# allegro/allRank

Hardware: AMD Instinct MI355X
Metric: slate-items/sec training (WEB30K synth, slate 240) (higher is better)
Workload: dtype f32 (split-bf16x3 contractions: GEMMs and attention); 1 GPU; WEB30K-synth F=136 L=240, fc[512] + 2x self-attention(d512,h8,d_ff2048) + ApproxNDCG (BASELINE configs[2]); slates_per_gpu=256, slate_len=240, global_batch=256, optimizer=Adam lr=1e-3, slates=dense, engine=fused, gemm=split_bf16, parallelism=slate-sharded dp1

## Files before the change

### allrank_amd/csrc/ltrx_mha.hip

```cpp
#include "ltrx_mfma.h"

using namespace ltrx;

namespace {

template <int DKP>
struct Tile {
  static constexpr int LDT = DKP + 4;
  static constexpr int FLOATS = 32 * LDT;
};

template <int DKP>
__device__ __forceinline__ void stage_tile(float* tile, const float* __restrict__ base, int row0, int nrows, int dk,
                                           size_t rs) {
  constexpr int C4 = DKP / 4;
  for (int idx = threadIdx.x; idx < 32 * C4; idx += blockDim.x) {
    const int r = idx / C4, c = (idx % C4) * 4;
    float4 v = make_float4(0.f, 0.f, 0.f, 0.f);
    if (row0 + r < nrows && c < dk) v = *reinterpret_cast<const float4*>(base + (size_t)(row0 + r) * rs + c);
    *reinterpret_cast<float4*>(tile + r * Tile<DKP>::LDT + c) = v;
  }
}

template <int DKP>
// ... 334 lines not shown
      del_t[threadIdx.x] = (qrow < L) ? delta[statb + qrow] : 0.f;
      if (DROP) drow_t[threadIdx.x] = drop_row_seed(drop, bh, Lmax, qrow);
    }
    __syncthreads();
    if (qt + 1 < nqt) {
      tile_gload<DKP>(qr, qb, (qt + 1) * 32, L, dk, rs);
      tile_gload<DKP>(dor, dob, (qt + 1) * 32, L, dk, ors);
    }
    const f32x16 s = rows_x_fixed<DKP>(qtile, kfrag);
    f32x16 p;
#pragma unroll
    for (int r = 0; r < 16; ++r) p[r] = fast_exp2(s[r] * sl2 + kbias - lse_t[rowmap(r, half)]);
    f32x16 dm;
#pragma unroll
    for (int r = 0; r < 16; ++r)
      dm[r] = DROP ? drop_scale_rk(drop, drow_t[rowmap(r, half)], key) : 1.0f;
    {
      f32x16 pd;
#pragma unroll
      for (int r = 0; r < 16; ++r) pd[r] = p[r] * dm[r];
      cols_x_p<DKP>(dotile, pd, dvacc);
    }
    const f32x16 dp = rows_x_fixed<DKP>(dotile, vfrag);
    f32x16 ds;
#pragma unroll
    for (int r = 0; r < 16; ++r) ds[r] = p[r] * (dp[r] * dm[r] - del_t[rowmap(r, half)]) * scale;
    cols_x_p<DKP>(qtile, ds, dkacc);
  }
  store_rows<DKP>(dkout + slate * drs + (size_t)head * dk, k0, L, dk, drs, dkacc, 1.0f);
  store_rows<DKP>(dvout + slate * drs + (size_t)head * dk, k0, L, dk, drs, dvacc, 1.0f);
}

__global__ void ltrx_selftest_mfma_kernel(const float* __restrict__ A, const float* __restrict__ Bm, float* __restrict__ D) {
  const int lane = threadIdx.x & 63, half = lane >> 5;
  f32x16 acc = {0.f, 0.f, 0.f, 0.f, 0.f, 0.f, 0.f, 0.f, 0.f, 0.f, 0.f, 0.f, 0.f, 0.f, 0.f, 0.f};
  acc = __builtin_amdgcn_mfma_f32_32x32x2f32(A[(lane & 31) * 2 + half], Bm[half * 32 + (lane & 31)], acc, 0, 0, 0);
  for (int r = 0; r < 16; ++r) D[rowmap(r, half) * 32 + (lane & 31)] = acc[r];
}

extern "C" int ltrx_selftest_mfma32x32x2(const float* A, const float* Bm, float* D, ltrx_stream_t stream) {
  if (!A || !Bm || !D) return LTRX_EINVAL;
  hipLaunchKernelGGL(ltrx_selftest_mfma_kernel, dim3(1), dim3(64), 0, (hipStream_t)stream, A, Bm, D);
  LTRX_LAUNCH_CHECK();
  return LTRX_OK;
}

bool ltrx_mha_res_fits(int L, int dk);
int ltrx_mha_fwd_res_launch(const float* q, const float* k, const float* v, const uint8_t* kpm, int B, int L, int h, int dk, int rs,
                            float* o, int ors, float* lse, float p_drop, uint32_t seed, const uint32_t* seed_step, const int* cu,
                            const int* order, bool plain, hipStream_t s);
int ltrx_mha_bwd_res_launch(const float* q, const float* k, const float* v, const uint8_t* kpm, const float* o, const float* dout,
                            const float* lse, int B, int L, int h, int dk, int rs, int ors, float* dq, float* dkk, float* dv, int drs,
                            void* ws, float p_drop, uint32_t seed, const uint32_t* seed_step, const int* cu, const int* order,
                            bool plain, hipStream_t s);
bool ltrx_mha_res_bwd_fits(int L, int dk);
size_t ltrx_mha_res_bwd_ws_bytes(int B, int L, int h);

static int mha_check(int B, int L, int h, int dk, int rs, int ors) {
  if (B <= 0 || L <= 0 || h <= 0 || dk <= 0) return LTRX_EINVAL;
  if (dk % 4 != 0 || dk > 128 || rs % 4 != 0 || ors % 4 != 0 || rs < h * dk || ors < h * dk) return LTRX_EUNSUPPORTED;
  if ((long long)B * h > 0x7fffffffLL || (L + 127) / 128 > 65535) return LTRX_EUNSUPPORTED;
  return LTRX_OK;
}

extern "C" int ltrx_mha_head_width_supported(int d_k) { return mha_check(1, 1, 1, d_k, d_k, d_k) == LTRX_OK ? 1 : 0; }

#define LTRX_DKP_DISPATCH(dk, CALL) \
  do {                              \
    if ((dk) <= 32) { CALL(32); }   \
    else if ((dk) <= 64) { CALL(64); } \
    else if ((dk) <= 96) { CALL(96); } \
    else { CALL(128); }             \
  } while (0)

static DropCfg make_drop(float p_drop, uint32_t seed) { return ltrx_make_drop(p_drop, seed); }

extern "C" int ltrx_mha_fwd(const float* q, const float* k, const float* v, const uint8_t* key_pad_mask, int B, int L,
                            int h, int d_k, int row_stride, float* o, int o_row_stride, float* lse_out, float p_drop,
                            uint32_t seed, const uint32_t* seed_step, const int32_t* cu_seqlens, const int32_t* slate_order,
                            int mode, ltrx_stream_t stream) {
  if (!q || !k || !v || (!key_pad_mask && !cu_seqlens) || !o || !lse_out || !(p_drop >= 0.f) || p_drop >= 1.f) return LTRX_EINVAL;
  if (mode < 0 || mode > 2) return LTRX_EINVAL;
  int rc = mha_check(B, L, h, d_k, row_stride, o_row_stride);
  if (rc != LTRX_OK) return rc;
  hipStream_t s = (hipStream_t)stream;
  if (mode != 0 && ltrx_mha_res_fits(L, d_k))
    return ltrx_mha_fwd_res_launch(q, k, v, key_pad_mask, B, L, h, d_k, row_stride, o, o_row_stride, lse_out, p_drop, seed, seed_step,
                                   cu_seqlens, slate_order, mode == 2, s);
  const DropCfg drop = make_drop(p_drop, seed);
  const dim3 grid(B * h, (L + 127) / 128);
  const float scale = 1.0f / sqrtf((float)d_k);
#define CALL(DKP)                                                                                                 \
  if (drop.thresh != 0u)                                                                                          \
    hipLaunchKernelGGL((ltrx_mha_fwd_kernel<DKP, true>), grid, dim3(256), 0, s, q, k, v, key_pad_mask, L, h, d_k, row_stride, \
                       o, o_row_stride, lse_out, scale, drop, seed_step, cu_seqlens, slate_order);                              \
  else                                                                                                            \
    hipLaunchKernelGGL((ltrx_mha_fwd_kernel<DKP, false>), grid, dim3(256), 0, s, q, k, v, key_pad_mask, L, h, d_k, row_stride, \
                       o, o_row_stride, lse_out, scale, drop, seed_step, cu_seqlens, slate_order)
  LTRX_DKP_DISPATCH(d_k, CALL);
#undef CALL
  LTRX_LAUNCH_CHECK();
  return LTRX_OK;
}

static bool res_bwd_selected(int B, int L, int h, int d_k) {
  return ltrx_mha_res_bwd_fits(L, d_k) && ltrx_mha_res_bwd_ws_bytes(B, L, h) <= (size_t)LTRX_MHA_DS_BUDGET_BYTES;
}

extern "C" size_t ltrx_mha_bwd_workspace_bytes(int B, int L, int h, int d_k, int mode) {
  if (B <= 0 || L <= 0 || h <= 0 || d_k <= 0) return 0;
  if (mode != 0 && res_bwd_selected(B, L, h, d_k)) return ltrx_mha_res_bwd_ws_bytes(B, L, h);
  return (size_t)B * L * h * sizeof(float);
}

extern "C" int ltrx_mha_bwd(const float* q, const float* k, const float* v, const uint8_t* key_pad_mask, const float* o,
                            const float* dout, const float* lse, int B, int L, int h, int d_k, int row_stride,
                            int o_row_stride, float* dq, float* dk, float* dv, int d_row_stride, float p_drop,
                            uint32_t seed, const uint32_t* seed_step, const int32_t* cu_seqlens, const int32_t* slate_order,
                            int mode, void* ws, ltrx_stream_t stream) {
  if (!q || !k || !v || (!key_pad_mask && !cu_seqlens) || !o || !dout || !lse || !dq || !dk || !dv || !ws) return LTRX_EINVAL;
  if (mode < 0 || mode > 2) return LTRX_EINVAL;
  if (!(p_drop >= 0.f) || p_drop >= 1.f) return LTRX_EINVAL;
  int rc = mha_check(B, L, h, d_k, row_stride, o_row_stride);
  if (rc != LTRX_OK) return rc;
  if (d_row_stride % 4 != 0 || d_row_stride < h * d_k) return LTRX_EUNSUPPORTED;
  hipStream_t s = (hipStream_t)stream;
  float* delta = (float*)ws;
  if (mode != 0 && res_bwd_selected(B, L, h, d_k))
    return ltrx_mha_bwd_res_launch(q, k, v, key_pad_mask, o, dout, lse, B, L, h, d_k, row_stride, o_row_stride, dq, dk, dv, d_row_stride,
                                   ws, p_drop, seed, seed_step, cu_seqlens, slate_order, mode == 2, s);
  const DropCfg drop = make_drop(p_drop, seed);
  const dim3 grid(B * h, (L + 127) / 128);
  const float scale = 1.0f / sqrtf((float)d_k);
#define CALLQ(DKP)                                                                                                   \
  if (drop.thresh != 0u)                                                                                             \
    hipLaunchKernelGGL((ltrx_mha_bwd_dq_kernel<DKP, true>), grid, dim3(256), 0, s, q, k, v, key_pad_mask, o, dout, lse, delta, \
                       L, h, d_k, row_stride, o_row_stride, dq, d_row_stride, scale, drop, seed_step, cu_seqlens, slate_order);    \
  else                                                                                                               \
    hipLaunchKernelGGL((ltrx_mha_bwd_dq_kernel<DKP, false>), grid, dim3(256), 0, s, q, k, v, key_pad_mask, o, dout, lse, delta, \
                       L, h, d_k, row_stride, o_row_stride, dq, d_row_stride, scale, drop, seed_step, cu_seqlens, slate_order)
  LTRX_DKP_DISPATCH(d_k, CALLQ);
#undef CALLQ
  LTRX_LAUNCH_CHECK();
#define CALLK(DKP)                                                                                                     \
  if (drop.thresh != 0u)                                                                                               \
    hipLaunchKernelGGL((ltrx_mha_bwd_dkdv_kernel<DKP, true>), grid, dim3(256), 0, s, q, k, v, key_pad_mask, dout, lse, delta, L, \
                       h, d_k, row_stride, o_row_stride, dk, dv, d_row_stride, scale, drop, seed_step, cu_seqlens, slate_order);      \
  else                                                                                                                 \
    hipLaunchKernelGGL((ltrx_mha_bwd_dkdv_kernel<DKP, false>), grid, dim3(256), 0, s, q, k, v, key_pad_mask, dout, lse, delta, L, \
                       h, d_k, row_stride, o_row_stride, dk, dv, d_row_stride, scale, drop, seed_step, cu_seqlens, slate_order)
  LTRX_DKP_DISPATCH(d_k, CALLK);
#undef CALLK
  LTRX_LAUNCH_CHECK();
  return LTRX_OK;
}
```

### allrank_amd/csrc/ltrx_mha_res.hip

```cpp
#include "ltrx_mfma.h"

using namespace ltrx;

namespace {

constexpr int RMAX = 256;
constexpr int DK = 64;
constexpr int PLANE = RMAX * DK * 2;
constexpr size_t RES_STATS = 4 * (size_t)PLANE + 3 * RMAX * sizeof(float);
constexpr int XROW = 64;
constexpr size_t dq_smem(int nw) { return 2 * (size_t)PLANE + (size_t)nw * 32 * 32 * sizeof(float); }
constexpr float kLog2e = 1.4426950408889634f;
constexpr float kLn2 = 0.6931471805599453f;


__device__ __forceinline__ int img_off(int row, int chunk) {
  const int s = ((row >> 2) & 1) | (((row >> 3) & 1) << 1) | (((row >> 1) & 1) << 2);
  return row * (DK * 2) + ((chunk ^ s) << 4);
}

struct TileRegs {
  float4 a, b;
};
__device__ __forceinline__ void tile_gload(TileRegs& r, const float* __restrict__ base, int tile, int nrows, int dk, size_t rs) {
// ... 23 lines not shown
  f32x4 x[8];
};
__device__ __forceinline__ void fixed_gload(FixedRegs& f, const float* __restrict__ base, int row0, int nrows, int dk, size_t rs) {
  const int lane = threadIdx.x & 63, c16 = lane & 15;
#pragma unroll
  for (int j = 0; j < 8; ++j) {
    const int r = (lane >> 4) + 4 * j;
    const bool ok = (row0 + r < nrows) && (4 * c16 < dk);
    const f32x4 v = *reinterpret_cast<const f32x4*>(base + (size_t)(ok ? row0 + r : 0) * rs + (ok ? 4 * c16 : 0));
    f.x[j] = ok ? v : f32x4{0.f, 0.f, 0.f, 0.f};
  }
}
__device__ __forceinline__ void fixed_finish(bf16x8 (&fh)[4], bf16x8 (&fl)[4], const FixedRegs& f, f32x4* scratch, float pre = 1.0f) {
  const int lane = threadIdx.x & 63, l31 = lane & 31, half = lane >> 5, c16 = lane & 15;
#pragma unroll
  for (int j = 0; j < 8; ++j) {
    const int r = (lane >> 4) + 4 * j;
    scratch[r * 16 + (c16 ^ (r & 15))] = f.x[j];
  }
#pragma unroll
  for (int ks = 0; ks < 4; ++ks) {
    const f32x4 a = scratch[l31 * 16 + ((4 * ks + 2 * half) ^ (l31 & 15))];
    const f32x4 b = scratch[l31 * 16 + ((4 * ks + 2 * half + 1) ^ (l31 & 15))];
    const float v[8] = {a.x * pre, a.y * pre, a.z * pre, a.w * pre, b.x * pre, b.y * pre, b.z * pre, b.w * pre};
#pragma unroll
    for (int e = 0; e < 8; ++e) {
      LTRX_SPLIT_BF16(v[e], fh[ks][e], fl[ks][e]);
    }
  }
}

#define LTRX_MFMA(a, b, c) __builtin_amdgcn_mfma_f32_32x32x16_bf16(a, b, c, 0, 0, 0)
#ifdef LTRX_MHA_STAMP
__device__ unsigned long long g_mha_stamps[8][40][8];
#define STAMP_(kt, ph)                                                                 \
  do {                                                                                 \
    __builtin_amdgcn_sched_barrier(0);                                                 \
    if (blockIdx.x == LTRX_MHA_STAMP && (threadIdx.x & 63) == 0) g_mha_stamps[threadIdx.x >> 6][kt][ph] = __builtin_readcyclecounter(); \
    __builtin_amdgcn_sched_barrier(0);                                                 \
  } while (0)
#ifdef LTRX_MHA_STAMP_DKDV
#define STAMP(kt, ph)
#define DSTAMP(kt, ph) STAMP_(kt, ph)
#else
#define STAMP(kt, ph) STAMP_(kt, ph)
#define DSTAMP(kt, ph)
#endif
#else
#define STAMP(kt, ph)
#define DSTAMP(kt, ph)
#endif
#ifndef LTRX_MHA_TOUCH
#define LTRX_MHA_TOUCH 1
#endif
#ifndef LTRX_MHA_PRIO_HALF
#define LTRX_MHA_PRIO_HALF 0
#endif

struct ColFrags {
  bf16x8 h[2][2], l[2][2];
};
__device__ __forceinline__ void store_rows(float* __restrict__ base, int row0, int nrows, int dk, size_t rs, const f32x16 (&out)[2],
                                           float scale, f32x4* scratch) {
  const int lane = threadIdx.x & 63, l31 = lane & 31, half = lane >> 5;
#pragma unroll
  for (int ct = 0; ct < 2; ++ct) {
#pragma unroll
    for (int g = 0; g < 4; ++g)
      scratch[l31 * 8 + ((2 * g + half) ^ ((l31 >> 1) & 7))] =
          f32x4{out[ct][4 * g + 0] * scale, out[ct][4 * g + 1] * scale, out[ct][4 * g + 2] * scale, out[ct][4 * g + 3] * scale};
#pragma unroll
    for (int j = 0; j < 4; ++j) {
      const int r = (lane >> 3) + 8 * j, c = 32 * ct + 4 * (lane & 7);
      const f32x4 v = scratch[r * 8 + ((lane & 7) ^ ((r >> 1) & 7))];
      if (row0 + r < nrows && c < dk) *reinterpret_cast<f32x4*>(base + (size_t)(row0 + r) * rs + c) = v;
    }
  }
}
__device__ __forceinline__ f32x4* end_scratch(unsigned char* smem, int last_tile, int wave) {
  const size_t half_off = (((last_tile & 7) >= 4) ? 0 : PLANE / 2);
  return reinterpret_cast<f32x4*>(smem + (size_t)(wave >> 2) * PLANE + half_off + (size_t)(wave & 3) * 4096);
}

__device__ __forceinline__ void zero2(f32x16 (&o)[2]) {
#pragma unroll
  for (int ct = 0; ct < 2; ++ct)
#pragma unroll
    for (int r = 0; r < 16; ++r) o[ct][r] = 0.f;
}

struct Slate {
  int b, head, bh, Lmax, len;
  size_t row0;
};
__device__ __forceinline__ Slate which_slate(int L, int h, const int* __restrict__ cu, const int* __restrict__ order) {
  Slate s;
  s.head = blockIdx.x % h;
  s.b = order ? order[blockIdx.x / h] : (int)(blockIdx.x / h);
  s.bh = s.b * h + s.head;
  s.Lmax = L;
  s.row0 = cu ? (size_t)cu[s.b] : (size_t)s.b * L;
  s.len = cu ? cu[s.b + 1] - cu[s.b] : L;
  return s;
}

struct Touch {
// ... 225 lines not shown
    const float mref = (mn == -INFINITY) ? 0.f : mn;
    if (__builtin_amdgcn_ballot_w64(grow) != 0) {
      const float alpha = grow ? fast_exp2(m - mref) : 1.0f;
      l *= alpha;
#pragma unroll
      for (int ct = 0; ct < 2; ++ct)
#pragma unroll
        for (int r = 0; r < 16; ++r) oacc[ct][r] *= alpha;
    }
    m = mn;
    f32x16 p;
    f32x2 ps2 = {0.f, 0.f};
    const f32x2 mref2 = {mref, mref};
#pragma unroll
    for (int r = 0; r < 16; r += 2) {
      const f32x2 t = f32x2{s[r], s[r + 1]} - mref2;
      const f32x2 e2 = {fast_exp2(t[0]), fast_exp2(t[1])};
      ps2 += e2;
      p[r] = e2[0];
      p[r + 1] = e2[1];
    }
    l += ps2[0] + ps2[1];
    if (DROP) {
#pragma unroll
      for (int r = 0; r < 16; ++r) p[r] *= drop_scale_rk(drop, drow, kt * 32 + rowmap(r, half));
    }
    STAMP(kt, 4);
    cols_mma<PL>(vimg + slot * (DK * 2), fo, p, oacc);
    STAMP(kt, 5);
  }
  STAMP(33, 0);
  if (!active) {
    if (LTRX_MHA_TOUCH) touch_join(tch);
    return;
  }
  const float lt = sum_across_halves(l);
  const float inv = (lt > 0.f) ? 1.0f / lt : 0.f;
  store_rows(o + sl.row0 * ors + (size_t)sl.head * dk, q0, len, dk, ors, oacc, inv, end_scratch(smem, nkt - 1, wave));
  const int qrow = q0 + (lane & 31);
  if (half == 0 && qrow < len) lse[((size_t)sl.b * h + sl.head) * sl.Lmax + qrow] = (lt > 0.f) ? (m + log2f(lt)) * kLn2 : 0.f;
  STAMP(34, 0);
  if (LTRX_MHA_TOUCH) touch_join(tch);
}

struct DsRegs {
  f32x4 x[4];
};
__device__ __forceinline__ void ds_gload(DsRegs& d, const float* __restrict__ rows, int tile, int LK) {
  const int lane = threadIdx.x & 63;
  const float* p = rows + (size_t)(lane >> 3) * LK + tile * 32 + (lane & 7) * 4;
#pragma unroll
  for (int j = 0; j < 4; ++j) d.x[j] = __builtin_nontemporal_load(reinterpret_cast<const f32x4*>(p + (size_t)(8 * j) * LK));
}
template <bool PL, int NW, int D, bool KPF>
__global__ void __launch_bounds__(64 * NW) __attribute__((amdgpu_waves_per_eu(2, 2))) ltrx_mha_bwd_dq_res_kernel(const float* __restrict__ k, const float* __restrict__ dsw, int LK, int L,
                                                                  int h, int dk, int rs, float* __restrict__ dq, int drs,
                                                                  const int* __restrict__ cu, const int* __restrict__ order) {
  extern __shared__ __attribute__((aligned(16))) unsigned char smem[];
  unsigned char* kimg = smem;
  const Slate sl = which_slate(L, h, cu, order);
  const int lane = threadIdx.x & 63, half = lane >> 5, wave = __builtin_amdgcn_readfirstlane(threadIdx.x >> 6), l31 = lane & 31;
  f32x4* xs = reinterpret_cast<f32x4*>(smem + 2 * PLANE) + wave * (32 * 32 / 4);
  const int len = sl.len;
  constexpr int TPT = 32 / NW;
  if ((int)(blockIdx.y * (32 * NW)) >= len) return;
  const float* src = k + sl.row0 * rs + (size_t)sl.head * dk;
  const int q0 = blockIdx.y * (32 * NW) + wave * 32;
  const int sub = (NW == 8) ? (int)(threadIdx.x >> 8) : 0;
  const bool active = q0 < len;
  const float* rows = dsw + ((size_t)sl.b * h + sl.head) * LK * LK + (size_t)q0 * LK;
  const int nkt = (len + 31) / 32, nchunk = KPF ? (nkt + 7) / 8 : 1;
  static_assert(KPF ? (8 % D == 0) : true, "the register slot of tile 8 c + s must not depend on c");
  TileRegs tr[TPT];
#pragma unroll
  for (int j = 0; j < TPT; ++j) tile_gload(tr[j], src, (8 / TPT) * j + sub, len, dk, rs);
  DsRegs dr[D];
  if (active) {
#pragma unroll
    for (int s = 0; s < D; ++s)
      if (s < nkt) ds_gload(dr[s], rows, s, LK);
  }
  f32x16 dqacc[2];
  zero2(dqacc);
  const TileOffsets fo = tile_offsets();
  for (int c = 0; c < nchunk; ++c) {
    if (c > 0) lds_only_barrier();
#pragma unroll
    for (int j = 0; j < TPT; ++j) tile_sstore<PL>(kimg, (8 / TPT) * j + sub, tr[j]);
    if (KPF && c + 1 < nchunk) {
#pragma unroll
      for (int j = 0; j < TPT; ++j) tile_gload(tr[j], src, 8 * (c + 1) + (8 / TPT) * j + sub, len, dk, rs);
    }
    lds_only_barrier();
    if (!active) continue;
#pragma unroll
    for (int s = 0; s < 8; ++s) {
      const int i = 8 * c + s;
      if (i >= nkt) break;
      DsRegs& cur = dr[s % D];
#pragma unroll
      for (int j = 0; j < 4; ++j) {
        const int r = (lane >> 3) + 8 * j;
        xs[r * 8 + ((lane & 7) ^ ((r >> 1) & 7))] = cur.x[j];
      }
      if (i + D < nkt) ds_gload(cur, rows, i + D, LK);
      f32x16 ds;
#pragma unroll
      for (int g = 0; g < 4; ++g) {
        const f32x4 x = xs[l31 * 8 + ((2 * g + half) ^ ((l31 >> 1) & 7))];
        ds[4 * g + 0] = x.x;
        ds[4 * g + 1] = x.y;
        ds[4 * g + 2] = x.z;
        ds[4 * g + 3] = x.w;
      }
      cols_mma<PL>(kimg + s * 32 * (DK * 2), fo, ds, dqacc);
    }
  }
  if (!active) return;
  store_rows(dq + sl.row0 * drs + (size_t)sl.head * dk, q0, len, dk, drs, dqacc, 1.0f, xs);
}

__device__ __forceinline__ float tile_delta(const TileRegs& g, const TileRegs& a) {
  float d = g.a.x * a.a.x + g.a.y * a.a.y + g.a.z * a.a.z + g.a.w * a.a.w;
  d += g.b.x * a.b.x + g.b.y * a.b.y + g.b.z * a.b.z + g.b.w * a.b.w;
  d += __shfl_xor(d, 4, 64);
  d += __shfl_xor(d, 2, 64);
  d += __shfl_xor(d, 1, 64);
  return d;
}
template <bool DROP, bool PL>
__global__ void __launch_bounds__(512) ltrx_mha_bwd_dkdv_res_kernel(
    const float* __restrict__ q, const float* __restrict__ k, const float* __restrict__ v, const uint8_t* __restrict__ kpm,
    const float* __restrict__ o, const float* __restrict__ dout, const float* __restrict__ lse, int L, int h, int dk, int rs, int ors,
    float* __restrict__ dkout, float* __restrict__ dvout, int drs, float* __restrict__ dsw, int LK, float scale, DropCfg drop,
    const uint32_t* __restrict__ drop_step, const int* __restrict__ cu, const int* __restrict__ order) {
  extern __shared__ __attribute__((aligned(16))) unsigned char smem[];
  unsigned char* qimg = smem;
  unsigned char* doimg = smem + 2 * PLANE;
  float* lse_t = reinterpret_cast<float*>(smem + 4 * PLANE);
  float* del_t = lse_t + RMAX;
  uint32_t* drow_t = reinterpret_cast<uint32_t*>(del_t + RMAX);
  if (DROP && drop_step) drop.seed ^= drop_step[0] * 0x9E3779B9u;
  const Slate sl = which_slate(L, h, cu, order);
  const int lane = threadIdx.x & 63, half = lane >> 5, wave = __builtin_amdgcn_readfirstlane(threadIdx.x >> 6);
  const int len = sl.len;
  const bool first = wave < 4;
  const float* src = first ? q + sl.row0 * rs + (size_t)sl.head * dk : dout + sl.row0 * ors + (size_t)sl.head * dk;
  const float* osrc = o + sl.row0 * ors + (size_t)sl.head * dk;
  const size_t srs = first ? (size_t)rs : (size_t)ors;
  unsigned char* dst = first ? qimg : doimg;
  TileRegs tr, to;
  DSTAMP(32, 0);
  tile_gload(tr, src, 0, len, dk, srs);
  if (!first) tile_gload(to, osrc, 0, len, dk, ors);
  const size_t statb = ((size_t)sl.b * h + sl.head) * sl.Lmax;
  float lse_n = 0.f;
  if (threadIdx.x < 32 && (int)threadIdx.x < len) lse_n = lse[statb + threadIdx.x];
  if ((int)(blockIdx.y * RMAX) >= len) return;
  const int k0 = blockIdx.y * RMAX + wave * 32;
  bf16x8 kh[4], kl[4], vh[4], vl[4];
  const bool active = k0 < len;
  const int key = k0 + (lane & 31);
  bool key_masked;
  {
    FixedRegs fk, fv;
    fixed_gload(fk, k + sl.row0 * rs + (size_t)sl.head * dk, k0, len, dk, rs);
    fixed_gload(fv, v + sl.row0 * rs + (size_t)sl.head * dk, k0, len, dk, rs);
    const uint8_t km = kpm ? kpm[sl.row0 + (key < len ? key : 0)] : (uint8_t)0;
    f32x4* scratch = reinterpret_cast<f32x4*>(smem + (size_t)(wave >> 1) * PLANE + PLANE / 2 + (size_t)(wave & 1) * 8192);
    fixed_finish(kh, kl, fk, scratch, scale * kLog2e);
    fixed_finish(vh, vl, fv, scratch, scale);
    key_masked = (key >= len) || km != 0;
  }
  const float kbias = key_masked ? -INFINITY : 0.f;
  const f32x2 kb2 = {kbias, kbias};
  const TileOffsets fo = tile_offsets();
  f32x16 dkacc[2], dvacc[2];
  zero2(dkacc);
  zero2(dvacc);
  const int nqt = (len + 31) / 32;
  if (LTRX_MHA_PRIO_HALF && wave >= 4) __builtin_amdgcn_s_setprio(1);
  float* const dsp = dsw + ((size_t)sl.b * h + sl.head) * LK * LK + (blockIdx.y * RMAX + wave * 32);
  const int dso = (4 * half * LK + (lane & 31)) * 4;
  DSTAMP(32, 1);
  for (int qt = 0; qt < nqt; ++qt) {
    DSTAMP(qt, 0);
    if (!first) {
      const float d = tile_delta(tr, to);
// ... 4 lines not shown
      const int qr = qt * 32 + threadIdx.x, sl_ = (qt & 7) * 32 + threadIdx.x;
      lse_t[sl_] = (qr < len) ? lse_n * kLog2e : INFINITY;
      if (DROP) drow_t[sl_] = drop_row_seed(drop, sl.bh, sl.Lmax, qr);
    }
    DSTAMP(qt, 1);
    lds_only_barrier();
    DSTAMP(qt, 2);
    if (!active) {
      if (qt + 1 < nqt) {
        tile_gload(tr, src, qt + 1, len, dk, srs);
        if (!first) tile_gload(to, osrc, qt + 1, len, dk, ors);
      }
      continue;
    }
    const int slot = (qt & 7) * 32;
    const unsigned char* qtile = qimg + slot * (DK * 2);
    const unsigned char* dotile = doimg + slot * (DK * 2);
    f32x16 p = rows_mma<PL>(qtile, fo, kh, kl);
    f32x16 ds = rows_mma<PL>(dotile, fo, vh, vl);
    DSTAMP(qt, 3);
    {
      const float* lse_p = reinterpret_cast<const float*>(reinterpret_cast<const unsigned char*>(lse_t + slot) + fo.kb);
      const float* del_p = reinterpret_cast<const float*>(reinterpret_cast<const unsigned char*>(del_t + slot) + fo.kb);
#pragma unroll
      for (int g = 0; g < 4; ++g) {
        const f32x4 ls4 = *reinterpret_cast<const f32x4*>(lse_p + 8 * g);
        const f32x4 dl4 = *reinterpret_cast<const f32x4*>(del_p + 8 * g);
#pragma unroll
        for (int e = 0; e < 4; e += 2) {
          const int r = 4 * g + e;
          const f32x2 t = (f32x2{p[r], p[r + 1]} - f32x2{ls4[e], ls4[e + 1]}) + kb2;
          const f32x2 pr = {fast_exp2(t[0]), fast_exp2(t[1])};
          f32x2 dm = {1.0f, 1.0f};
          if (DROP) {
            const int qr = slot + rowmap(r, half);
            dm = f32x2{drop_scale_rk(drop, drow_t[qr], key), drop_scale_rk(drop, drow_t[qr + 1], key)};
          }
          const f32x2 dpv = {ds[r], ds[r + 1]};
          const f32x2 x = (DROP ? dpv * dm : dpv) - f32x2{dl4[e], dl4[e + 1]};
          const f32x2 dsv = pr * x;
          const f32x2 pm = DROP ? pr * dm : pr;
          ds[r] = dsv[0];
          ds[r + 1] = dsv[1];
          p[r] = pm[0];
          p[r + 1] = pm[1];
        }
      }
    }
    DSTAMP(qt, 4);
    {
      const float* const t = dsp + (size_t)(qt * 32) * LK;
#pragma unroll
      for (int r = 0; r < 16; ++r)
        asm volatile("global_store_dword %0, %1, %2 nt" ::"v"(dso), "v"(ds[r]), "s"(t + (size_t)((r & 3) + 8 * (r >> 2)) * LK));
    }
    __builtin_amdgcn_sched_barrier(0);
    if (qt + 1 < nqt) {
      tile_gload(tr, src, qt + 1, len, dk, srs);
      if (!first) tile_gload(to, osrc, qt + 1, len, dk, ors);
      if (threadIdx.x < 32 && (qt + 1) * 32 + (int)threadIdx.x < len) lse_n = lse[statb + (qt + 1) * 32 + threadIdx.x];
    }
    DSTAMP(qt, 5);
    __builtin_amdgcn_sched_barrier(0);
    cols_mma<PL>(dotile, fo, p, dvacc);
    DSTAMP(qt, 6);
    __builtin_amdgcn_sched_barrier(0);
    cols_mma<PL>(qtile, fo, ds, dkacc);
    DSTAMP(qt, 7);
    __builtin_amdgcn_sched_barrier(0);
  }
  DSTAMP(33, 0);
  if (!active) return;
  f32x4* const es = end_scratch(smem, nqt - 1, wave);
  store_rows(dkout + sl.row0 * drs + (size_t)sl.head * dk, k0, len, dk, drs, dkacc, 1.0f, es);
  store_rows(dvout + sl.row0 * drs + (size_t)sl.head * dk, k0, len, dk, drs, dvacc, 1.0f, es);
  DSTAMP(34, 0);
}

static constexpr size_t RES_SMEM = RES_STATS;

bool ltrx_mha_res_fits(int L, int dk) { return L > 0 && (L + RMAX - 1) / RMAX <= 65535 && dk > 32 && dk <= DK; }
bool ltrx_mha_res_bwd_fits(int L, int dk) { return ltrx_mha_res_fits(L, dk) && L <= LTRX_MAX_SLATE_LEN; }
static int ds_stride(int L) { return (L + XROW - 1) / XROW * XROW; }
size_t ltrx_mha_res_bwd_ws_bytes(int B, int L, int h) {
  const size_t lk = (size_t)ds_stride(L);
  return (size_t)B * h * lk * lk * sizeof(float);
}

int ltrx_mha_fwd_res_launch(const float* q, const float* k, const float* v, const uint8_t* kpm, int B, int L, int h, int dk, int rs,
                            float* o, int ors, float* lse, float p_drop, uint32_t seed, const uint32_t* seed_step, const int* cu,
                            const int* order, bool plain, hipStream_t s) {
  static std::atomic<uint64_t> attr_done{0};
  const int arc = ltrx_allow_dynamic_lds(attr_done, {{ltrx_mha_fwd_res_kernel<false, false>, RES_SMEM}, {ltrx_mha_fwd_res_kernel<true, false>, RES_SMEM},
                                                     {ltrx_mha_fwd_res_kernel<false, true>, RES_SMEM}, {ltrx_mha_fwd_res_kernel<true, true>, RES_SMEM}});
  if (arc != LTRX_OK) return arc;
  const DropCfg drop = ltrx_make_drop(p_drop, seed);
  const float scale = 1.0f / sqrtf((float)dk);
  const dim3 grid(B * h, (L + RMAX - 1) / RMAX);
#define LTRX_FWD(D_, P_)                                                                                                          \
  hipLaunchKernelGGL((ltrx_mha_fwd_res_kernel<D_, P_>), grid, dim3(512), RES_SMEM, s, q, k, v, kpm, L, h, dk, rs, o, ors, lse, scale, \
                     drop, seed_step, cu, order)
  if (drop.thresh != 0u) {
    if (plain) LTRX_FWD(true, true); else LTRX_FWD(true, false);
  } else {
    if (plain) LTRX_FWD(false, true); else LTRX_FWD(false, false);
  }
#undef LTRX_FWD
  LTRX_LAUNCH_CHECK();
  return LTRX_OK;
}

int ltrx_mha_bwd_res_launch(const float* q, const float* k, const float* v, const uint8_t* kpm, const float* o, const float* dout,
                            const float* lse, int B, int L, int h, int dk, int rs, int ors, float* dq, float* dkk, float* dv, int drs,
                            void* ws, float p_drop, uint32_t seed, const uint32_t* seed_step, const int* cu, const int* order,
                            bool plain, hipStream_t s) {
  static std::atomic<uint64_t> attr_done{0};
  const int arc = ltrx_allow_dynamic_lds(
      attr_done, {{ltrx_mha_bwd_dq_res_kernel<false, 4, 6, false>, dq_smem(4)}, {ltrx_mha_bwd_dq_res_kernel<true, 4, 6, false>, dq_smem(4)},
                  {ltrx_mha_bwd_dq_res_kernel<false, 8, 4, true>, dq_smem(8)}, {ltrx_mha_bwd_dq_res_kernel<true, 8, 4, true>, dq_smem(8)},
                  {ltrx_mha_bwd_dkdv_res_kernel<false, false>, RES_SMEM}, {ltrx_mha_bwd_dkdv_res_kernel<true, false>, RES_SMEM},
                  {ltrx_mha_bwd_dkdv_res_kernel<false, true>, RES_SMEM}, {ltrx_mha_bwd_dkdv_res_kernel<true, true>, RES_SMEM}});
  if (arc != LTRX_OK) return arc;
  const DropCfg drop = ltrx_make_drop(p_drop, seed);
  const float scale = 1.0f / sqrtf((float)dk);
  const dim3 grid(B * h, (L + RMAX - 1) / RMAX);
  const int LK = ds_stride(L);
  float* dsw = (float*)ws;
#define LTRX_DKDV(D_, P_)                                                                                                          \
  hipLaunchKernelGGL((ltrx_mha_bwd_dkdv_res_kernel<D_, P_>), grid, dim3(512), RES_SMEM, s, q, k, v, kpm, o, dout, lse, L, h, dk,  \
                     rs, ors, dkk, dv, drs, dsw, LK, scale, drop, seed_step, cu, order)
  if (drop.thresh != 0u) {
    if (plain) LTRX_DKDV(true, true); else LTRX_DKDV(true, false);
  } else {
    if (plain) LTRX_DKDV(false, true); else LTRX_DKDV(false, false);
  }
#undef LTRX_DKDV
  LTRX_LAUNCH_CHECK();
#define LTRX_DQ(P_, NW_, D_, K_)                                                                                                   \
  hipLaunchKernelGGL((ltrx_mha_bwd_dq_res_kernel<P_, NW_, D_, K_>), dim3(B * h, (L + 32 * NW_ - 1) / (32 * NW_)), dim3(64 * NW_),      \
                     dq_smem(NW_), s, k, dsw, LK, L, h, dk, rs, dq, drs, cu, order)
  if (grid.y == 1) {
    if (plain) LTRX_DQ(true, 4, 6, false); else LTRX_DQ(false, 4, 6, false);
  } else {
    if (plain) LTRX_DQ(true, 8, 4, true); else LTRX_DQ(false, 8, 4, true);
  }
#undef LTRX_DQ
  LTRX_LAUNCH_CHECK();
  return LTRX_OK;
}

#ifdef LTRX_MHA_STAMP
extern "C" int ltrx_debug_mha_stamps(unsigned long long* host_dst) {
  return hipMemcpyFromSymbol(host_dst, HIP_SYMBOL(g_mha_stamps), sizeof(unsigned long long) * 8 * 40 * 8) == hipSuccess ? 0 : 1;
}
#endif
```

### include/ltrx.h

```cpp
#ifndef LTRX_H
#define LTRX_H

#include <stddef.h>
#include <stdint.h>

#ifdef __cplusplus
extern "C" {
#endif

#define LTRX_VERSION 130

#define LTRX_OK 0
#define LTRX_EINVAL (-1)
#define LTRX_EUNSUPPORTED (-2)
#define LTRX_EHIP (-1000)

#define LTRX_MAX_SLATE_LEN 2048
#define LTRX_MAX_LONG_SLATE_LEN 16384
#define LTRX_MHA_DS_BUDGET_BYTES (2147483648ull)
#define LTRX_MAX_METRIC_SLATE_LEN 8192

typedef void* ltrx_stream_t;

int ltrx_version(void);
// ... 73 lines not shown

size_t ltrx_binary_listnet_workspace_bytes(int B, int L);
int ltrx_binary_listnet_fwd_bwd(const float* y_pred, const float* y_true, int B, int L, float eps, float pad_value,
                                float batch_divisor, float* loss_out, float* grad_out, void* ws, ltrx_stream_t stream);

size_t ltrx_mrr_workspace_bytes(int B, int L, int n_ats);
int ltrx_mrr_at(const float* y_pred, const float* y_true, int B, int L, const int* ats, int n_ats, float pad_value,
                float* mrr_out, void* ws, ltrx_stream_t stream);

int ltrx_listnet_fwd_bwd_cu(const float* y_pred, const float* y_true, const int32_t* cu_seqlens, const int32_t* slate_order, int B,
                            int max_len, float eps, float batch_divisor, float* loss_out, float* per_slate_out, float* grad_out,
                            void* ws, ltrx_stream_t stream);
int ltrx_approxndcg_fwd_bwd_cu(const float* y_pred, const float* y_true, const int32_t* cu_seqlens, const int32_t* slate_order, int B,
                               int max_len, float eps, float alpha, float batch_divisor, float* loss_out, float* per_slate_out,
                               float* grad_out, void* ws, ltrx_stream_t stream);
int ltrx_lambdaloss_fwd_bwd_cu(const float* y_pred, const float* y_true, const int32_t* cu_seqlens, const int32_t* slate_order, int B,
                               int max_len, float eps, int scheme, int k, float sigma, float mu, int reduction, int logbase,
                               const float* ext_pair_count, float* loss_out, float* pair_count_out, float* grad_out,
                               int64_t* order_out, void* ws, ltrx_stream_t stream);
int ltrx_ndcg_at_cu(const float* y_pred, const float* y_true, const int32_t* cu_seqlens, const int32_t* slate_order, int B,
                    int max_len, const int* ats, int n_ats, float filler_value, float* ndcg_out, float* dcg_out, int64_t* order_out,
                    void* ws, ltrx_stream_t stream);
int ltrx_mrr_at_cu(const float* y_pred, const float* y_true, const int32_t* cu_seqlens, const int32_t* slate_order, int B, int max_len,
                   const int* ats, int n_ats, float* mrr_out, void* ws, ltrx_stream_t stream);


int ltrx_layernorm_fwd(const float* x, const float* res, const float* a, const float* b, int rows, int D, float eps,
                       float* xsum_out, float* y_out, float* mean_out, float* rstd_out, float res_drop_p, uint32_t drop_seed,
                       const uint32_t* drop_step, ltrx_stream_t stream);
size_t ltrx_layernorm_bwd_workspace_bytes(int rows, int D);
int ltrx_layernorm_bwd(const float* dy, const float* xsum, const float* a, const float* mean, const float* rstd,
                       const float* dres_in, int rows, int D, float eps, float* dx_out, float* da_out, float* db_out,
                       void* ws, ltrx_stream_t stream);
int ltrx_layernorm_bwd_partial(const float* dy, const float* xsum, const float* a, const float* mean, const float* rstd,
                               const float* dres_in, int rows, int D, float eps, float* dx_out, void* ws, int* partial_rows_out,
                               ltrx_stream_t stream);

int ltrx_norm_head_fwd(const float* x, const float* a, const float* b, const float* w, const float* bias, int rows, int D, float eps,
                       float* scores_out, float* mean_out, float* rstd_out, float* y_out, ltrx_stream_t stream);
size_t ltrx_norm_head_bwd_workspace_bytes(int rows, int D);
int ltrx_norm_head_bwd_partial(const float* dscores, const float* xsum, const float* a, const float* w, const float* mean,
                               const float* rstd, int rows, int D, float eps, float* dx_out, void* ws, int* partial_rows_out,
                               ltrx_stream_t stream);
int ltrx_norm_head_wgrad(const float* dscores, const float* xsum, const float* a, const float* b, const float* mean, const float* rstd,
                         int M, int D, float* dw, float* db, void* ws, ltrx_stream_t stream);

#define LTRX_MHA_EXACT_FP32 0
#define LTRX_MHA_SPLIT_BF16 1
#define LTRX_MHA_PLAIN_BF16 2
int ltrx_mha_fwd(const float* q, const float* k, const float* v, const uint8_t* key_pad_mask, int B, int L, int h,
                 int d_k, int row_stride, float* o, int o_row_stride, float* lse_out, float p_drop, uint32_t seed,
                 const uint32_t* seed_step, const int32_t* cu_seqlens, const int32_t* slate_order, int mode,
                 ltrx_stream_t stream);
size_t ltrx_mha_bwd_workspace_bytes(int B, int L, int h, int d_k, int mode);
int ltrx_mha_head_width_supported(int d_k);
int ltrx_mha_bwd(const float* q, const float* k, const float* v, const uint8_t* key_pad_mask, const float* o,
                 const float* dout, const float* lse, int B, int L, int h, int d_k, int row_stride, int o_row_stride,
                 float* dq, float* dk, float* dv, int d_row_stride, float p_drop, uint32_t seed,
                 const uint32_t* seed_step, const int32_t* cu_seqlens, const int32_t* slate_order, int mode, void* ws,
                 ltrx_stream_t stream);


int ltrx_adam_step(float* params, const float* grads, float* exp_avg, float* exp_avg_sq, size_t n, float lr, float beta1,
                   float beta2, float eps, float weight_decay, int decoupled, float* step_count, float grad_scale,
                   const float* grad_scale_dev, ltrx_stream_t stream);
int ltrx_sgd_step(float* params, const float* grads, float* momentum_buf, size_t n, float lr, float momentum, int nesterov,
                  float weight_decay, float grad_scale, const float* grad_scale_dev, ltrx_stream_t stream);

size_t ltrx_clip_workspace_bytes(size_t n);
int ltrx_clip_grad_norm_scale(const float* grads, size_t n, float max_norm, float* scale_out, float* norm_out, void* ws,
                              ltrx_stream_t stream);

size_t ltrx_colsum_workspace_bytes(int M, int N);
int ltrx_colsum(const float* a, int M, int N, int ld, float* out, int accumulate, void* ws, ltrx_stream_t stream);

int ltrx_relu_bwd(float* dr_inout, const float* r_post_act, size_t n, float scale, ltrx_stream_t stream);

int ltrx_dropout_apply(const float* src, float* dst, size_t n, float p, uint32_t seed, const uint32_t* drop_step,
                       ltrx_stream_t stream);
int ltrx_bump_u32(uint32_t* word, ltrx_stream_t stream);

int ltrx_first_nonfinite(const float* buf, size_t n, const int64_t* seg_start, int n_seg, int* out, ltrx_stream_t stream);

int ltrx_transpose_batch(const float* src_base, float* dst_base, const int64_t* desc, const int32_t* tile_start, int n,
                         int total_tiles, ltrx_stream_t stream);

int ltrx_gather_rows(const float* src, int ld_src, const int32_t* idx, int n, int n_pad, int cols, float* dst, int ld_dst,
                     ltrx_stream_t stream);
int ltrx_packed_row_index(const int32_t* cu_seqlens, int B, int L, int n, int32_t* idx, ltrx_stream_t stream);
int ltrx_scatter_rows(const float* src, int ld_src, const int32_t* idx, int n, int cols, float* dst, int ld_dst,
                      ltrx_stream_t stream);

int ltrx_assemble_packed(const float* x_items, const float* y_items, const int64_t* offsets, const int64_t* slates,
                         const int32_t* cu_seqlens, int B, int L, int F, int rows, float* x_out, int ld_x, float* y_out,
                         int32_t* idx_out, int64_t* pos_out, ltrx_stream_t stream);
int ltrx_gather_rows_cu(const float* src, int ld_src, const int32_t* cu_seqlens, int B, int L, int cols, int rows, float* dst,
                        int ld_dst, int32_t* idx_out, ltrx_stream_t stream);
int ltrx_scatter_rows_cu(const float* src, int ld_src, const int32_t* cu_seqlens, int B, int L, int cols, int rows, float* dst,
                         int ld_dst, ltrx_stream_t stream);

int ltrx_score_head_fwd(const float* x, const float* w, const float* b, int M, int D, float* scores, ltrx_stream_t stream);
size_t ltrx_score_head_bwd_workspace_bytes(int M, int D);
int ltrx_score_head_bwd(const float* dscores, const float* x, const float* w, int M, int D, float* dx, float* dw,
                        float* db, void* ws, ltrx_stream_t stream);

size_t ltrx_gemm_nt_relu_bits_bytes(int M, int N, int K);
// ... 81 lines not shown
```

Before: 7.310 million slate-items/s.

## Fuse dQ computation into dK/dV residual backward kernel for single-tile slates

When the whole slate fits in one row tile (grid.y==1), the dK/dV backward kernel now goes on to compute dQ itself. It reuses its LDS to stage K and reads back the dS rows it just wrote, so the separate dQ kernel launch is skipped. The aim is to remove a launch and the cross-kernel round trip through the dS workspace. In exchange, each block keeps more registers live for the prefetch buffers and gains an extra barrier and serialized tail work. A mode flag keeps the old two-launch path available, and the fused path is disabled for dropout in non-plain mode.

```diff
diff --git a/allrank_amd/csrc/ltrx_mha.hip b/allrank_amd/csrc/ltrx_mha.hip
--- a/allrank_amd/csrc/ltrx_mha.hip
+++ b/allrank_amd/csrc/ltrx_mha.hip
@@ -410,7 +410,7 @@
 int ltrx_mha_bwd_res_launch(const float* q, const float* k, const float* v, const uint8_t* kpm, const float* o, const float* dout,
                             const float* lse, int B, int L, int h, int dk, int rs, int ors, float* dq, float* dkk, float* dv, int drs,
                             void* ws, float p_drop, uint32_t seed, const uint32_t* seed_step, const int* cu, const int* order,
-                            bool plain, hipStream_t s);
+                            bool plain, bool two_launches, hipStream_t s);
 bool ltrx_mha_res_bwd_fits(int L, int dk);
 size_t ltrx_mha_res_bwd_ws_bytes(int B, int L, int h);
 
@@ -467,6 +467,7 @@
 
 extern "C" size_t ltrx_mha_bwd_workspace_bytes(int B, int L, int h, int d_k, int mode) {
   if (B <= 0 || L <= 0 || h <= 0 || d_k <= 0) return 0;
+  mode &= ~LTRX_MHA_BWD_TWO_LAUNCHES;
   if (mode != 0 && res_bwd_selected(B, L, h, d_k)) return ltrx_mha_res_bwd_ws_bytes(B, L, h);
   return (size_t)B * L * h * sizeof(float);
 }
@@ -477,6 +478,8 @@
                             uint32_t seed, const uint32_t* seed_step, const int32_t* cu_seqlens, const int32_t* slate_order,
                             int mode, void* ws, ltrx_stream_t stream) {
   if (!q || !k || !v || (!key_pad_mask && !cu_seqlens) || !o || !dout || !lse || !dq || !dk || !dv || !ws) return LTRX_EINVAL;
+  const bool two_launches = mode >= 0 && (mode & LTRX_MHA_BWD_TWO_LAUNCHES) != 0;
+  if (two_launches) mode &= ~LTRX_MHA_BWD_TWO_LAUNCHES;
   if (mode < 0 || mode > 2) return LTRX_EINVAL;
   if (!(p_drop >= 0.f) || p_drop >= 1.f) return LTRX_EINVAL;
   int rc = mha_check(B, L, h, d_k, row_stride, o_row_stride);
@@ -486,7 +489,7 @@
   float* delta = (float*)ws;
   if (mode != 0 && res_bwd_selected(B, L, h, d_k))
     return ltrx_mha_bwd_res_launch(q, k, v, key_pad_mask, o, dout, lse, B, L, h, d_k, row_stride, o_row_stride, dq, dk, dv, d_row_stride,
-                                   ws, p_drop, seed, seed_step, cu_seqlens, slate_order, mode == 2, s);
+                                   ws, p_drop, seed, seed_step, cu_seqlens, slate_order, mode == 2, two_launches, s);
   const DropCfg drop = make_drop(p_drop, seed);
   const dim3 grid(B * h, (L + 127) / 128);
   const float scale = 1.0f / sqrtf((float)d_k);
diff --git a/allrank_amd/csrc/ltrx_mha_res.hip b/allrank_amd/csrc/ltrx_mha_res.hip
--- a/allrank_amd/csrc/ltrx_mha_res.hip
+++ b/allrank_amd/csrc/ltrx_mha_res.hip
@@ -99,6 +99,9 @@
 #endif
 #ifndef LTRX_MHA_TOUCH
 #define LTRX_MHA_TOUCH 1
+#endif
+#ifndef LTRX_MHA_DS_STORE
+#define LTRX_MHA_DS_STORE " nt"
 #endif
 #ifndef LTRX_MHA_PRIO_HALF
 #define LTRX_MHA_PRIO_HALF 0
@@ -430,6 +433,29 @@
 #pragma unroll
   for (int j = 0; j < 4; ++j) d.x[j] = __builtin_nontemporal_load(reinterpret_cast<const f32x4*>(p + (size_t)(8 * j) * LK));
 }
+#define LTRX_DS_PREFETCH(D_, dr_)              \
+  _Pragma("unroll") for (int s = 0; s < D_; ++s) \
+    if (s < nkt) ds_gload(dr_[s], rows, s, LK);
+#define LTRX_DQ_CHUNK(PL_, D_, dr_, c_, dqacc_)                                                                         \
+  _Pragma("unroll") for (int s = 0; s < 8; ++s) {                                                                       \
+    const int i = 8 * (c_) + s;                                                                                         \
+    if (i >= nkt) break;                                                                                                \
+    DsRegs& cur = dr_[s % D_];                                                                     \
+    _Pragma("unroll") for (int j = 0; j < 4; ++j) {                                                                     \
+      const int r = (lane >> 3) + 8 * j;                                                                                \
+      xs[r * 8 + ((lane & 7) ^ ((r >> 1) & 7))] = cur.x[j];                                                             \
+    }                                                                                                                   \
+    if (i + D_ < nkt) ds_gload(cur, rows, i + D_, LK);                                                                  \
+    f32x16 ds;                                                                                                          \
+    _Pragma("unroll") for (int g = 0; g < 4; ++g) {                                                                     \
+      const f32x4 x = xs[l31 * 8 + ((2 * g + half) ^ ((l31 >> 1) & 7))];        \
+      ds[4 * g + 0] = x.x;                                                                                              \
+      ds[4 * g + 1] = x.y;                                                                                              \
+      ds[4 * g + 2] = x.z;                                                                                              \
+      ds[4 * g + 3] = x.w;                                                                                              \
+    }                                                                                                                   \
+    cols_mma<PL_>(kimg + s * 32 * (DK * 2), fo, ds, dqacc_);          \
+  }
 template <bool PL, int NW, int D, bool KPF>
 __global__ void __launch_bounds__(64 * NW) __attribute__((amdgpu_waves_per_eu(2, 2))) ltrx_mha_bwd_dq_res_kernel(const float* __restrict__ k, const float* __restrict__ dsw, int LK, int L,
                                                                   int h, int dk, int rs, float* __restrict__ dq, int drs,
@@ -454,9 +480,7 @@
   for (int j = 0; j < TPT; ++j) tile_gload(tr[j], src, (8 / TPT) * j + sub, len, dk, rs);
   DsRegs dr[D];
   if (active) {
-#pragma unroll
-    for (int s = 0; s < D; ++s)
-      if (s < nkt) ds_gload(dr[s], rows, s, LK);
+    LTRX_DS_PREFETCH(D, dr)
   }
   f32x16 dqacc[2];
   zero2(dqacc);
@@ -471,28 +495,7 @@
     }
     lds_only_barrier();
     if (!active) continue;
-#pragma unroll
-    for (int s = 0; s < 8; ++s) {
-      const int i = 8 * c + s;
-      if (i >= nkt) break;
-      DsRegs& cur = dr[s % D];
-#pragma unroll
-      for (int j = 0; j < 4; ++j) {
-        const int r = (lane >> 3) + 8 * j;
-        xs[r * 8 + ((lane & 7) ^ ((r >> 1) & 7))] = cur.x[j];
-      }
-      if (i + D < nkt) ds_gload(cur, rows, i + D, LK);
-      f32x16 ds;
-#pragma unroll
-      for (int g = 0; g < 4; ++g) {
-        const f32x4 x = xs[l31 * 8 + ((2 * g + half) ^ ((l31 >> 1) & 7))];
-        ds[4 * g + 0] = x.x;
-        ds[4 * g + 1] = x.y;
-        ds[4 * g + 2] = x.z;
-        ds[4 * g + 3] = x.w;
-      }
-      cols_mma<PL>(kimg + s * 32 * (DK * 2), fo, ds, dqacc);
-    }
+    LTRX_DQ_CHUNK(PL, D, dr, c, dqacc)
   }
   if (!active) return;
   store_rows(dq + sl.row0 * drs + (size_t)sl.head * dk, q0, len, dk, drs, dqacc, 1.0f, xs);
@@ -506,12 +509,13 @@
   d += __shfl_xor(d, 1, 64);
   return d;
 }
-template <bool DROP, bool PL>
+constexpr int FUSED_D = 6;
+template <bool DROP, bool PL, bool DQ>
 __global__ void __launch_bounds__(512) ltrx_mha_bwd_dkdv_res_kernel(
     const float* __restrict__ q, const float* __restrict__ k, const float* __restrict__ v, const uint8_t* __restrict__ kpm,
     const float* __restrict__ o, const float* __restrict__ dout, const float* __restrict__ lse, int L, int h, int dk, int rs, int ors,
     float* __restrict__ dkout, float* __restrict__ dvout, int drs, float* __restrict__ dsw, int LK, float scale, DropCfg drop,
-    const uint32_t* __restrict__ drop_step, const int* __restrict__ cu, const int* __restrict__ order) {
+    const uint32_t* __restrict__ drop_step, const int* __restrict__ cu, const int* __restrict__ order, float* __restrict__ dqout) {
   extern __shared__ __attribute__((aligned(16))) unsigned char smem[];
   unsigned char* qimg = smem;
   unsigned char* doimg = smem + 2 * PLANE;
@@ -622,7 +626,7 @@
       const float* const t = dsp + (size_t)(qt * 32) * LK;
 #pragma unroll
       for (int r = 0; r < 16; ++r)
-        asm volatile("global_store_dword %0, %1, %2 nt" ::"v"(dso), "v"(ds[r]), "s"(t + (size_t)((r & 3) + 8 * (r >> 2)) * LK));
+        asm volatile("global_store_dword %0, %1, %2" LTRX_MHA_DS_STORE ::"v"(dso), "v"(ds[r]), "s"(t + (size_t)((r & 3) + 8 * (r >> 2)) * LK));
     }
     __builtin_amdgcn_sched_barrier(0);
     if (qt + 1 < nqt) {
@@ -640,11 +644,44 @@
     __builtin_amdgcn_sched_barrier(0);
   }
   DSTAMP(33, 0);
-  if (!active) return;
-  f32x4* const es = end_scratch(smem, nqt - 1, wave);
-  store_rows(dkout + sl.row0 * drs + (size_t)sl.head * dk, k0, len, dk, drs, dkacc, 1.0f, es);
-  store_rows(dvout + sl.row0 * drs + (size_t)sl.head * dk, k0, len, dk, drs, dvacc, 1.0f, es);
-  DSTAMP(34, 0);
+  if constexpr (!DQ) {
+    if (!active) return;
+    f32x4* const es = end_scratch(smem, nqt - 1, wave);
+    store_rows(dkout + sl.row0 * drs + (size_t)sl.head * dk, k0, len, dk, drs, dkacc, 1.0f, es);
+    store_rows(dvout + sl.row0 * drs + (size_t)sl.head * dk, k0, len, dk, drs, dvacc, 1.0f, es);
+    DSTAMP(34, 0);
+  } else {
+    asm volatile("s_waitcnt vmcnt(0)" ::: "memory");
+    __syncthreads();
+    DSTAMP(35, 0);
+    unsigned char* const kimg = smem;
+    f32x4* const xs = reinterpret_cast<f32x4*>(smem + 2 * PLANE) + wave * (32 * 32 / 4);
+    const float* const ksrc = k + sl.row0 * rs + (size_t)sl.head * dk;
+    const int sub = (int)(threadIdx.x >> 8);
+    TileRegs kr[4];
+#pragma unroll
+    for (int j = 0; j < 4; ++j) tile_gload(kr[j], ksrc, 2 * j + sub, len, dk, rs);
+    const float* const rows = dsw + ((size_t)sl.b * h + sl.head) * LK * LK + (size_t)k0 * LK;
+    const int l31 = lane & 31, nkt = nqt;
+    DsRegs dr[FUSED_D];
+    if (active) {
+      LTRX_DS_PREFETCH(FUSED_D, dr)
+      store_rows(dkout + sl.row0 * drs + (size_t)sl.head * dk, k0, len, dk, drs, dkacc, 1.0f, xs);
+      store_rows(dvout + sl.row0 * drs + (size_t)sl.head * dk, k0, len, dk, drs, dvacc, 1.0f, xs);
+    }
+    DSTAMP(34, 0);
+#pragma unroll
+    for (int j = 0; j < 4; ++j) tile_sstore<PL>(kimg, 2 * j + sub, kr[j]);
+    lds_only_barrier();
+    DSTAMP(36, 0);
+    if (!active) return;
+    f32x16 dqacc[2];
+    zero2(dqacc);
+    LTRX_DQ_CHUNK(PL, FUSED_D, dr, 0, dqacc)
+    DSTAMP(37, 0);
+    store_rows(dqout + sl.row0 * drs + (size_t)sl.head * dk, k0, len, dk, drs, dqacc, 1.0f, xs);
+    DSTAMP(38, 0);
+  }
 }
 
 static constexpr size_t RES_SMEM = RES_STATS;
@@ -683,22 +720,36 @@
 int ltrx_mha_bwd_res_launch(const float* q, const float* k, const float* v, const uint8_t* kpm, const float* o, const float* dout,
                             const float* lse, int B, int L, int h, int dk, int rs, int ors, float* dq, float* dkk, float* dv, int drs,
                             void* ws, float p_drop, uint32_t seed, const uint32_t* seed_step, const int* cu, const int* order,
-                            bool plain, hipStream_t s) {
+                            bool plain, bool two_launches, hipStream_t s) {
   static std::atomic<uint64_t> attr_done{0};
   const int arc = ltrx_allow_dynamic_lds(
-      attr_done, {{ltrx_mha_bwd_dq_res_kernel<false, 4, 6, false>, dq_smem(4)}, {ltrx_mha_bwd_dq_res_kernel<true, 4, 6, false>, dq_smem(4)},
+      attr_done, {{ltrx_mha_bwd_dkdv_res_kernel<false, false, true>, RES_SMEM}, {ltrx_mha_bwd_dkdv_res_kernel<false, true, true>, RES_SMEM},
+                  {ltrx_mha_bwd_dkdv_res_kernel<true, true, true>, RES_SMEM},
+                  {ltrx_mha_bwd_dq_res_kernel<false, 4, 6, false>, dq_smem(4)}, {ltrx_mha_bwd_dq_res_kernel<true, 4, 6, false>, dq_smem(4)},
                   {ltrx_mha_bwd_dq_res_kernel<false, 8, 4, true>, dq_smem(8)}, {ltrx_mha_bwd_dq_res_kernel<true, 8, 4, true>, dq_smem(8)},
-                  {ltrx_mha_bwd_dkdv_res_kernel<false, false>, RES_SMEM}, {ltrx_mha_bwd_dkdv_res_kernel<true, false>, RES_SMEM},
-                  {ltrx_mha_bwd_dkdv_res_kernel<false, true>, RES_SMEM}, {ltrx_mha_bwd_dkdv_res_kernel<true, true>, RES_SMEM}});
+                  {ltrx_mha_bwd_dkdv_res_kernel<false, false, false>, RES_SMEM}, {ltrx_mha_bwd_dkdv_res_kernel<true, false, false>, RES_SMEM},
+                  {ltrx_mha_bwd_dkdv_res_kernel<false, true, false>, RES_SMEM}, {ltrx_mha_bwd_dkdv_res_kernel<true, true, false>, RES_SMEM}});
   if (arc != LTRX_OK) return arc;
   const DropCfg drop = ltrx_make_drop(p_drop, seed);
   const float scale = 1.0f / sqrtf((float)dk);
   const dim3 grid(B * h, (L + RMAX - 1) / RMAX);
   const int LK = ds_stride(L);
   float* dsw = (float*)ws;
+  const bool dropping = drop.thresh != 0u;
+  if (grid.y == 1 && !two_launches && !(dropping && !plain)) {
+#define LTRX_FUSED(D_, P_)                                                                                                         \
+  hipLaunchKernelGGL((ltrx_mha_bwd_dkdv_res_kernel<D_, P_, true>), grid, dim3(512), RES_SMEM, s, q, k, v, kpm, o, dout, lse, L, h, dk, \
+                     rs, ors, dkk, dv, drs, dsw, LK, scale, drop, seed_step, cu, order, dq)
+    if (!plain) LTRX_FUSED(false, false);
+    else if (dropping) LTRX_FUSED(true, true);
+    else LTRX_FUSED(false, true);
+#undef LTRX_FUSED
+    LTRX_LAUNCH_CHECK();
+    return LTRX_OK;
+  }
 #define LTRX_DKDV(D_, P_)                                                                                                          \
-  hipLaunchKernelGGL((ltrx_mha_bwd_dkdv_res_kernel<D_, P_>), grid, dim3(512), RES_SMEM, s, q, k, v, kpm, o, dout, lse, L, h, dk,  \
-                     rs, ors, dkk, dv, drs, dsw, LK, scale, drop, seed_step, cu, order)
+  hipLaunchKernelGGL((ltrx_mha_bwd_dkdv_res_kernel<D_, P_, false>), grid, dim3(512), RES_SMEM, s, q, k, v, kpm, o, dout, lse, L, h, dk, \
+                     rs, ors, dkk, dv, drs, dsw, LK, scale, drop, seed_step, cu, order, (float*)nullptr)
   if (drop.thresh != 0u) {
     if (plain) LTRX_DKDV(true, true); else LTRX_DKDV(true, false);
   } else {
diff --git a/include/ltrx.h b/include/ltrx.h
--- a/include/ltrx.h
+++ b/include/ltrx.h
@@ -149,6 +149,7 @@
                  int d_k, int row_stride, float* o, int o_row_stride, float* lse_out, float p_drop, uint32_t seed,
                  const uint32_t* seed_step, const int32_t* cu_seqlens, const int32_t* slate_order, int mode,
                  ltrx_stream_t stream);
+#define LTRX_MHA_BWD_TWO_LAUNCHES 0x100
 size_t ltrx_mha_bwd_workspace_bytes(int B, int L, int h, int d_k, int mode);
 int ltrx_mha_head_width_supported(int d_k);
 int ltrx_mha_bwd(const float* q, const float* k, const float* v, const uint8_t* key_pad_mask, const float* o,
```

After: 7.363 million slate-items/s, median of 6. About the same (+0.7%).
